# MariBax/self-supervised-depth-estimation

Measured on AMD Instinct MI355X. Metric: training images/sec at 192x640 bs12 (resnet18 depth+pose, 4-scale photometric+smoothness), higher is better.
Workload: dtype f32 (1x1 convolutions: bf16x3 split operands, fp32 accumulate); 1 GPU; BASELINE configs[1]: resnet18 depth+pose, 192x640, per-GPU batch 12, 4 scales, frames {0,-1,+1}, automasking, Adam lr 1e-4; random-init weights; global_batch=12, parallelism=dp1, tiebreak_noise=on-device counter RNG, setup_steps=0, step_launch=eager (one launch per kernel)

## Files before the change

### include/depthcore.h

```cpp
#ifndef DEPTHCORE_H
#define DEPTHCORE_H

#include <stddef.h>
#include <stdint.h>

#ifdef __cplusplus
extern "C" {
#endif

#define DC_OK 0
#define DC_EINVAL (-1)
#define DC_ELAUNCH (-2)
#define DC_EWORKSPACE (-3)
#define DC_EEMPTY (-4)

#define DC_MAX_SCALES 4

#define DC_OPT_NO_AUTOMASK 1u
#define DC_OPT_AVG_REPROJ 2u
#define DC_OPT_NO_SSIM 4u
#define DC_OPT_ALIGN_CORNERS 8u
#define DC_OPT_PRED_MASK 32u
#define DC_OPT_PHOTO_SPLIT 64u
#define DC_OPT_PHOTO_FULL 128u
// ... 312 lines not shown
} dc_attn_map;
typedef struct dc_attn_params {
    const float *wq, *bq, *wk, *bk, *wv, *bv, *rel_h, *rel_w;
} dc_attn_params;
int dc_attnconv_fwd(const dc_attn_map* x, const dc_attn_params* p, const dc_attn_map* res, float* y, int B, int C, int H, int W,
                    int relu_in, int relu_res, void* stream);
int dc_attnconv_param_count(int C);
size_t dc_attnconv_bwd_workspace(int B, int C, int H, int W);
int dc_attnconv_bwd(const dc_attn_map* x, const dc_attn_params* p, const dc_attn_map* res, const float* gy, const dc_attn_map* dx,
                    const float* dx_add, const dc_attn_map* dres, float* dparams, void* ws, int B, int C, int H, int W, int relu_in,
                    int relu_res, void* stream);

int dc_sasa_plan(int B, int C, int H, int W, int* plan);
int dc_sasa_fwd(const float* q, const float* k, const float* v, long long q_bstride, long long k_bstride, long long v_bstride,
                const float* rel_h, const float* rel_w, float* y, float* lse, int B, int C, int H, int W, void* stream);
size_t dc_sasa_bwd_workspace(int B, int C, int H, int W);
int dc_sasa_bwd(const float* q, const float* k, const float* v, long long q_bstride, long long k_bstride, long long v_bstride,
                const float* rel_h, const float* rel_w, const float* y, const float* lse, const float* gy, float* dq, float* dk,
                float* dv, float* drel_h, float* drel_w, void* ws, int B, int C, int H, int W, void* stream);

int dc_gru_rh_fwd(const float* gates, const float* h, float* rh, int B, int C, int P, void* stream);
int dc_gru_rh_bwd(const float* gates, const float* h, const float* g, float* d_gates, float* d_h, int B, int C, int P, void* stream);
int dc_gru_blend_fwd(const float* gates, const float* h, const float* cnm, float* h_next, int B, int C, int P, void* stream);
int dc_gru_blend_bwd(const float* gates, const float* h, const float* cnm, const float* g, float* d_gates, float* d_h, float* d_cnm,
                     int B, int C, int P, void* stream);
int dc_gru_rh_bwd_acc(const float* gates, const float* h, const float* g, float* d_gates, float* d_h, int B, int C, int P, void* stream);
int dc_gru_blend_bwd_acc(const float* gates, const float* h, const float* cnm, const float* g, float* d_gates, float* d_h, float* d_cnm,
                         int B, int C, int P, void* stream);
int dc_gather_copy(const float* const* src, float* const* dst, const size_t* n, int nseg, void* stream);
int dc_gru_residual_fwd(const float* f, const float* H, float* out, int n, size_t M, void* stream);
int dc_gru_residual_bwd(const float* g, float* d_H, int n, size_t M, void* stream);

typedef struct dc_gru_infer_level {
    const float* gates;
    const float* cnm;
    const float* f;
    float* h;
    float* rh;
    float* out;
    int32_t C, P;
} dc_gru_infer_level;
int dc_gru_infer_rh(const dc_gru_infer_level* lv, int nlev, int B, void* stream);
int dc_gru_infer_tail(const dc_gru_infer_level* lv, int nlev, int B, void* stream);
int dc_gru_infer_init(const float* const* h0, float* const* state, const size_t* M, int nlev, int B, void* stream);

enum { DC_PREC_F32 = 0, DC_PREC_BF16 = 1 };
int dc_set_matrix_precision(int precision);
int dc_get_matrix_precision(void);

int dc_set_wino_f4(int mode);
int dc_set_wino_persist(int mode);
#define DC_WINO_PHASE_DEFAULT (-3)
int dc_set_wino_phase(int mode);
int dc_set_dgrad_split(int mode);
int dc_wino_cache_new_owner(void);
int dc_wino_cache_register(int owner, const float* weight, int Ci, int Co);
int dc_wino_cache_release_owner(int owner);
int dc_wino_cache_refresh(int owner, void* stream);
int dc_wino_cache_invalidate(int owner);
int dc_wino_cache_clear(void);
int dc_wino_cache_variants(void);

#define DC_JITTER_NONE (-1)
#define DC_JITTER_BRIGHTNESS 0
#define DC_JITTER_CONTRAST 1
#define DC_JITTER_SATURATION 2
#define DC_JITTER_HUE 3
int dc_resample_ksize(int in_size, int out_size);
int dc_resample_table(int in_size, int out_size, int* bounds, int* kk);
int dc_data_resize_axis(const uint8_t* src, uint8_t* dst, int n_img, int Hi, int Wi, int out_size, int axis, const int* bounds,
                        const int* kk, int ksize, const uint8_t* flip, void* stream);
int dc_data_flip(const uint8_t* src, uint8_t* dst, int n_img, int H, int W, const uint8_t* flip, void* stream);
int dc_data_jitter(uint8_t* img, int n_img, int npix, const int* steps, const float* params, unsigned long long* sums, void* stream);
int dc_data_to_tensor(const uint8_t* img, float* out, int n_img, int npix, void* stream);
int dc_data_jitter_to_tensor(const uint8_t* img, float* color, float* color_aug, int n_img, int npix, const int* steps,
                             const float* params, unsigned long long* sums, void* stream);
int dc_data_to_rgbx(const uint8_t* img, float* out, int n_img, int npix, void* stream);
int dc_pack_rgbx(const float* x, float* out, int n_img, int npix, void* stream);
typedef struct dc_ragged_img {
    long long src_off, dst_off;
    int Hi, Wi, table, flip;
} dc_ragged_img;
typedef struct dc_ragged_table {
    int bounds_off, kk_off, ksize, in_size;
} dc_ragged_table;
int dc_data_ragged_resize_axis(const uint8_t* src, size_t src_bytes, uint8_t* dst, size_t dst_bytes, const dc_ragged_img* desc_host,
                               const dc_ragged_img* desc_dev, int n_img, int out_size, int axis, const dc_ragged_table* tab_host,
                               const dc_ragged_table* tab_dev, int n_tab, const int* bounds_host, const int* bounds_dev,
                               size_t bounds_len, const int* kk_dev, size_t kk_len, void* stream);
typedef struct dc_cached_img {
    long long slot_off;
    int flip, reserved;
} dc_cached_img;
int dc_data_cached_levels(const uint8_t* arena, size_t arena_bytes, const dc_cached_img* desc_host, const dc_cached_img* desc_dev,
                          int n_img, int height, int width, int num_scales, float* const* color, float* const* color_aug,
                          float* packed, const int* steps, const float* params, unsigned long long* sums, void* stream);
typedef struct dc_seq_plan {
    long long lds_bytes, table_len, scratch_bytes;
    int n_img, tail_start;
} dc_seq_plan;
int dc_data_seq_plan(int n, int H, int W, int S, int jitter, int lds_budget, dc_seq_plan* plan);
int dc_data_seq_levels(const uint8_t* frames, int n, int H, int W, int S, int flip, float* const* color, float* packed,
                       const int* steps, const float* params, const int* tab_host, const int* tab_dev, size_t tab_len,
                       void* scratch, size_t scratch_bytes, int lds_budget, void* stream);

#define DC_EVAL_TRAINER 0
// ... 53 lines not shown
```

### self-supervised-depth-estimation_amd/csrc/wino_wgrad.hip

```cpp
#include "dc_common.h"
#include "conv_bf16.h"
#include "conv_prof.h"
#include "wino.h"

#include <algorithm>

namespace dc {

using f4 = __attribute__((ext_vector_type(4))) float;
using f2w = __attribute__((ext_vector_type(2))) float;
using wrsrc_t = __amdgpu_buffer_rsrc_t;

constexpr int WG_MR = 4, WG_KR = 2;
constexpr int WG_KT = 16 * WG_KR;
constexpr int WG_GPS = 66;
constexpr int WG_XPS = 130;
constexpr int WINO_PHASES = 2;
constexpr int WG_SLAB = 4 * WG_MR * WG_KR * 4 * 3 * 64;

struct WinoWgArgs {
    const float* x; const float* gy; float* slab;
    int B, K, M, H, W;
    const float* x1;
    int C0, up0, pad;
    unsigned x1bytes;
    int RH, RW, GRS, XRS;
    int regs_x, regs_y, nsub;
    int splits, kblocks, mblocks;
    unsigned xbytes, gbytes;
    unsigned mg_nmk, mg_kblocks, mg_RW, mg_XPR, mg_per_img, mg_regs_x;
    unsigned long long* diag;
    const float* in_scale; const float* in_shift;
    int npg;
    int phase;
};
unsigned long long* wino_diag_ptr();

template <bool FUSED, int MR, int NG, int BNIN = 0>
__global__ __launch_bounds__(256 * NG, 2) void wino_wgrad_kernel(WinoWgArgs a) {
    static_assert(!(FUSED && BNIN), "the BatchNorm fold exists for the plain trunk launches");
    constexpr int KR = WG_KR, MT = 16 * MR, NGQ = MT / 8;
    constexpr int GL = MT * WG_GPS, XL = WG_KT * WG_XPS, GROUP_LDS = 2 * GL + 2 * XL;
    static_assert(NG == 1 || NG * GROUP_LDS >= 4 * MR * KR * 4 * 3 * 64, "the q exchange aliases the staging slabs");
    extern __shared__ float wg_smem[];
#ifdef WINO_DIAG
    const unsigned long long dg_start = __builtin_amdgcn_s_memtime(), dg_rstart = __builtin_amdgcn_s_memrealtime();
#endif
    const int lane = threadIdx.x & 63, wave_all = __builtin_amdgcn_readfirstlane(threadIdx.x >> 6);
    const int grp = NG == 1 ? 0 : wave_all >> 2, wave = wave_all & 3, tid = threadIdx.x & 255;
    int early = 0;
    if constexpr (NG == 2) {
        const int phase = a.phase < 0 ? (grp == 1 ? 0 : WINO_PHASES - 1) : a.phase;
        early = __builtin_amdgcn_readfirstlane(phase == 0 ? 1 : 0);
    }
    float* const gl0 = wg_smem + grp * GROUP_LDS;
    float* const xl0 = gl0 + 2 * GL;
    auto gl = [&](int buf) { return gl0 + buf * GL; };
    auto xl = [&](int buf) { return xl0 + buf * XL; };
    const int cl = lane & 15, tq = lane >> 4;
    const int H = a.H, W = a.W, RH = a.RH, RW = a.RW, GRS = a.GRS, XRS = a.XRS;
    const int nmk = a.mblocks * a.kblocks;
    const int lbid = xcd_logical_block(blockIdx.x, gridDim.x);
    const int split0 = fdiv(lbid, a.mg_nmk), mk = lbid - split0 * nmk;
    const int mb = fdiv(mk, a.mg_kblocks), kb = mk - mb * a.kblocks;
    const int per_img = a.regs_x * a.regs_y;
    const unsigned plane = (unsigned)(H * W) * 4u;
    const wrsrc_t gr = __builtin_amdgcn_make_buffer_rsrc(const_cast<float*>(a.gy), (short)0, (int)a.gbytes, 0x00020000);
    const wrsrc_t xr = __builtin_amdgcn_make_buffer_rsrc(const_cast<float*>(a.x), (short)0, (int)a.xbytes, 0x00020000);
    const wrsrc_t x1r = __builtin_amdgcn_make_buffer_rsrc(const_cast<float*>(FUSED ? a.x1 : a.x), (short)0,
                                                          (int)(FUSED ? a.x1bytes : a.xbytes), 0x00020000);
    const int C0 = FUSED ? a.C0 : a.K, up0 = FUSED ? a.up0 : 0;
    const unsigned plane0 = up0 ? (unsigned)((H >> 1) * (W >> 1)) * 4u : plane;

    const int gslot = tid & 31, gcg = tid >> 5;
    const int grow = fdiv(gslot, a.mg_RW), gcp = gslot - grow * RW;
    const bool g_in = gslot < 2 * RH * RW;
    const int glds = gcg * WG_GPS + grow * GRS + 2 * gcp;
    const int xslot = tid & 63, xcg = tid >> 6;
    const int XPR = RW + 2;
    const int xrow = fdiv(xslot, a.mg_XPR), xcp = xslot - xrow * XPR;
    const bool x_in = xslot < (2 * RH + 2) * XPR;
    const int xlds0 = xcg * WG_XPS + xrow * XRS + max(2 * xcp - 1, 0), xlds1 = xcg * WG_XPS + xrow * XRS + 2 * xcp;

    f2w pg[NGQ], px[8];
    bool px_ok = false;
    int px_grp = 0;
    float bsc[BNIN == 2 ? 2 : 1][BNIN ? 8 : 1], bsh[BNIN == 2 ? 2 : 1][BNIN ? 8 : 1];
    if constexpr (BNIN != 0) {
#pragma unroll
        for (int q = 0; q < 8; ++q) {
            const int chc = min(kb * WG_KT + wave + 4 * q, a.K - 1);
// ... 116 lines not shown
            for (int i = 0; i < MR; ++i) {
                if (i + 1 < MR) {
                    graw[(i + 1) & 1][0] = *reinterpret_cast<const f2w*>(gs_ + (i + 1) * 16 * WG_GPS + goffA[ks]);
                    graw[(i + 1) & 1][1] = *reinterpret_cast<const f2w*>(gs_ + (i + 1) * 16 * WG_GPS + goffB[ks]);
                }
                __builtin_amdgcn_sched_barrier(0);
                float r0 = fmaf(graw[i & 1][1].x, gs, graw[i & 1][0].x);
                float r1 = fmaf(graw[i & 1][1].y, gs, graw[i & 1][0].y);
                r0 = tv ? r0 : 0.f;
                r1 = tv ? r1 : 0.f;
                const float d1 = r0 + r1, d2 = r0 - r1;
#pragma unroll
                for (int j = 0; j < KR; ++j) {
                    acc[i][j][0] = __builtin_amdgcn_mfma_f32_16x16x4f32(r0, v[j][0], acc[i][j][0], 0, 0, 0);
                    acc[i][j][1] = __builtin_amdgcn_mfma_f32_16x16x4f32(d1, v[j][1], acc[i][j][1], 0, 0, 0);
                    acc[i][j][2] = __builtin_amdgcn_mfma_f32_16x16x4f32(d2, v[j][2], acc[i][j][2], 0, 0, 0);
                    acc[i][j][3] = __builtin_amdgcn_mfma_f32_16x16x4f32(r1, v[j][3], acc[i][j][3], 0, 0, 0);
                }
                __builtin_amdgcn_sched_barrier(0);
            }
        }
    };

    const int stride = NG * a.splits;
    int sub = split0 + grp * a.splits;
    if (sub < a.nsub) {
        prefetch(sub);
        commit(0);
        if (sub + stride < a.nsub) prefetch(sub + stride);
    }
    __syncthreads();
    if (early && sub + stride < a.nsub) {
        commit(1);
        if (sub + 2 * stride < a.nsub) prefetch(sub + 2 * stride);
    }
#ifdef WINO_DIAG
    const unsigned long long dg0 = __builtin_amdgcn_s_memtime();
#endif
    for (int it = 0, lead = split0; lead < a.nsub; lead += stride, sub += stride, ++it) {
        if (sub < a.nsub) compute(it & 1);
        if (early) __syncthreads();
        const int nxt = sub + (1 + early) * stride;
        if (nxt < a.nsub) {
            commit((it + 1 + early) & 1);
            if (nxt + stride < a.nsub) prefetch(nxt + stride);
        }
        if (!early) __syncthreads();
    }

#ifdef WINO_DIAG
    const unsigned long long dg1 = __builtin_amdgcn_s_memtime();
#endif
    const float sa = wave == 3 ? -1.f : 1.f;
    float* dst = a.slab + ((size_t)(split0 * nmk + mk) * 4 + wave) * (MR * KR * 4 * 3 * 64) + lane;
    float* ex = wg_smem + (size_t)wave * (MR * KR * 4 * 3 * 64) + lane;
    if (NG == 2 && grp == 1) {
#pragma unroll
        for (int i = 0; i < MR; ++i)
#pragma unroll
            for (int j = 0; j < KR; ++j)
#pragma unroll
                for (int r = 0; r < 4; ++r) {
                    const float u0 = sa * acc[i][j][0][r], u1 = sa * acc[i][j][1][r], u2 = sa * acc[i][j][2][r];
                    const float u3 = -sa * acc[i][j][3][r];
                    const float h = 0.5f * (u1 + u2);
                    float* d = ex + (((i * KR + j) * 4 + r) * 3) * 64;
                    d[0] = u0 + h;
                    d[64] = 0.5f * (u1 - u2);
                    d[128] = h + u3;
                }
    }
    if (NG == 2) __syncthreads();
    if (grp == 0) {
#pragma unroll
        for (int i = 0; i < MR; ++i)
#pragma unroll
            for (int j = 0; j < KR; ++j)
#pragma unroll
                for (int r = 0; r < 4; ++r) {
                    const float u0 = sa * acc[i][j][0][r], u1 = sa * acc[i][j][1][r], u2 = sa * acc[i][j][2][r];
                    const float u3 = -sa * acc[i][j][3][r];
                    const float h = 0.5f * (u1 + u2);
                    const int e = (((i * KR + j) * 4 + r) * 3) * 64;
                    float q0 = u0 + h, q1 = 0.5f * (u1 - u2), q2 = h + u3;
                    if (NG == 2) { q0 += ex[e]; q1 += ex[e + 64]; q2 += ex[e + 128]; }
                    dst[e] = q0;
                    dst[e + 64] = q1;
                    dst[e + 128] = q2;
                }
    }
#ifdef WINO_DIAG
    if (a.diag && lane == 0 && wave_all == 0) {
        __builtin_amdgcn_s_waitcnt(0x0f70);
        unsigned long long* o = a.diag + (size_t)blockIdx.x * 8;
        unsigned hwid, xcc;
        asm volatile("s_getreg_b32 %0, hwreg(HW_REG_HW_ID)" : "=s"(hwid));
        asm volatile("s_getreg_b32 %0, hwreg(HW_REG_XCC_ID)" : "=s"(xcc));
        o[1] = hwid; o[2] = xcc; o[3] = 0; o[4] = dg1 - dg0; o[5] = dg0 - dg_start;
        o[6] = __builtin_amdgcn_s_memtime() - dg1; o[7] = dg_rstart;
        o[0] = __builtin_amdgcn_s_memrealtime();
    }
#endif
}

constexpr int WR_GROUPS = 16;
__global__ __launch_bounds__(64 * WR_GROUPS) void wino_wreduce_kernel(const float* __restrict__ slab, float* __restrict__ dw,
                                                                      int splits, int nmk, int kblocks, int M, int K, int MR) {
    constexpr int KR = WG_KR;
    const size_t WAVE_SLAB = (size_t)MR * KR * 4 * 3 * 64;
    __shared__ float part[WR_GROUPS][12][64];
    const int lane = threadIdx.x & 63, grp = threadIdx.x >> 6;
    int e = blockIdx.x;
    const int r = e & 3; e >>= 2;
    const int j = e % KR; e /= KR;
    const int i = e % MR; e /= MR;
    const int mk = e;
    float q[4][3];
#pragma unroll
    for (int w = 0; w < 4; ++w)
#pragma unroll
        for (int c = 0; c < 3; ++c) q[w][c] = 0.f;
    const int groups = blockDim.x >> 6;
    const int per = (splits + groups - 1) / groups;
    const int s1 = min(splits, (grp + 1) * per);
    for (int s = grp * per; s < s1; ++s) {
        const float* src = slab + ((size_t)(s * nmk + mk) * 4) * WAVE_SLAB + (size_t)(((i * KR + j) * 4 + r) * 3) * 64 + lane;
#pragma unroll
        for (int w = 0; w < 4; ++w)
#pragma unroll
            for (int c = 0; c < 3; ++c) q[w][c] += src[(size_t)w * WAVE_SLAB + c * 64];
    }
#pragma unroll
    for (int w = 0; w < 4; ++w)
#pragma unroll
        for (int c = 0; c < 3; ++c) part[grp][w * 3 + c][lane] = q[w][c];
    __syncthreads();
    if (grp != 0) return;
#pragma unroll
    for (int w = 0; w < 4; ++w)
#pragma unroll
        for (int c = 0; c < 3; ++c) {
            float t = part[0][w * 3 + c][lane];
            for (int g = 1; g < groups; ++g) t += part[g][w * 3 + c][lane];
            q[w][c] = t;
        }
    const int mbk = mk / kblocks, kbk = mk - mbk * kblocks;
    const int m = mbk * (16 * MR) + i * 16 + (lane >> 4) * 4 + r, k = kbk * WG_KT + j * 16 + (lane & 15);
    if (m >= M || k >= K) return;
    float* out = dw + ((size_t)m * K + k) * 9;
#pragma unroll
    for (int c = 0; c < 3; ++c) {
        const float h = 0.5f * (q[1][c] + q[2][c]);
        out[0 + c] = q[0][c] + h;
        out[3 + c] = 0.5f * (q[1][c] - q[2][c]);
        out[6 + c] = h + q[3][c];
    }
}

__global__ __launch_bounds__(64 * WR_GROUPS) void wino_wreduce_col_kernel(const float* __restrict__ slab, float* __restrict__ dw,
                                                                      int splits, int nmk, int kblocks, int M, int K, int MR) {
    constexpr int KR = WG_KR;
    const size_t WAVE_SLAB = (size_t)MR * KR * 4 * 3 * 64;
    __shared__ float part[WR_GROUPS][4][64];
    const int lane = threadIdx.x & 63, grp = threadIdx.x >> 6;
    int e = blockIdx.x;
    const int c = e % 3; e /= 3;
    const int r = e & 3; e >>= 2;
    const int j = e % KR; e /= KR;
    const int i = e % MR; e /= MR;
    const int mk = e;
    float q[4] = {0.f, 0.f, 0.f, 0.f};
    const int groups = blockDim.x >> 6;
    const int per = (splits + groups - 1) / groups;
    const int s1 = min(splits, (grp + 1) * per);
    for (int s = grp * per; s < s1; ++s) {
        const float* src = slab + ((size_t)(s * nmk + mk) * 4) * WAVE_SLAB + (size_t)(((i * KR + j) * 4 + r) * 3 + c) * 64 + lane;
#pragma unroll
        for (int w = 0; w < 4; ++w) q[w] += src[(size_t)w * WAVE_SLAB];
    }
#pragma unroll
    for (int w = 0; w < 4; ++w) part[grp][w][lane] = q[w];
    __syncthreads();
    if (grp != 0) return;
#pragma unroll
    for (int w = 0; w < 4; ++w) {
        float t = part[0][w][lane];
        for (int g = 1; g < groups; ++g) t += part[g][w][lane];
        q[w] = t;
    }
    const int mbk = mk / kblocks, kbk = mk - mbk * kblocks;
    const int m = mbk * (16 * MR) + i * 16 + (lane >> 4) * 4 + r, k = kbk * WG_KT + j * 16 + (lane & 15);
    if (m >= M || k >= K) return;
    float* out = dw + ((size_t)m * K + k) * 9;
    const float h = 0.5f * (q[1] + q[2]);
    out[0 + c] = q[0] + h;
    out[3 + c] = 0.5f * (q[1] - q[2]);
    out[6 + c] = h + q[3];
}

static constexpr size_t wg_lds(int mr, int ng) { return (size_t)ng * (2 * 16 * mr * WG_GPS + 2 * WG_KT * WG_XPS) * sizeof(float); }

struct WgKernel { void (*fn)(WinoWgArgs); int threads; size_t lds; };
template <bool FUSED, int MR, int NG, int BNIN = 0>
static constexpr WgKernel wg_kernel() { return {wino_wgrad_kernel<FUSED, MR, NG, BNIN>, 256 * NG, wg_lds(MR, NG)}; }
enum { WG_ROW_FUSED = 3 };
static const WgKernel g_wg_kernels[4 * 3] = {
    wg_kernel<false, 4, 1>(), wg_kernel<false, 4, 2>(), wg_kernel<false, 2, 1>(),
    wg_kernel<false, 4, 1, 1>(), wg_kernel<false, 4, 2, 1>(), wg_kernel<false, 2, 1, 1>(),
    wg_kernel<false, 4, 1, 2>(), wg_kernel<false, 4, 2, 2>(), wg_kernel<false, 2, 1, 2>(),
    wg_kernel<true, 4, 1>(), wg_kernel<true, 4, 2>(), wg_kernel<true, 2, 1>(),
};

constexpr int WG_PHASE_SHIPPED = -1;
static bool wino_phase_valid(int m) { return m == DC_WINO_PHASE_DEFAULT || (m >= -1 && m < WINO_PHASES); }
static int g_wino_phase = [] {
    const char* f = getenv("DC_WINO_PHASE");
    const int v = f ? atoi(f) : DC_WINO_PHASE_DEFAULT;
    return wino_phase_valid(v) ? v : DC_WINO_PHASE_DEFAULT;
}();

struct WgPlan { int RH, RW, GRS, XRS, regs_x, regs_y, nsub, mblocks, kblocks, splits, mr, ng; };

static WgPlan wg_plan(int B, int Ci, int Co, int H, int W) {
    WgPlan p{};
    const int TH = ceil_div(H, 2), TW = W / 2;
    const int cand[3][4] = {{2, 8, 16, 20}, {4, 4, 8, 12}, {3, 5, 10, 14}};
    double best = -1.0;
    for (auto& c : cand) {
        const double util = (double)TH * TW / ((double)ceil_div(TH, c[0]) * ceil_div(TW, c[1]) * 16.0);
        if (util > best + 1e-9) { best = util; p.RH = c[0]; p.RW = c[1]; p.GRS = c[2]; p.XRS = c[3]; }
    }
    p.regs_x = ceil_div(TW, p.RW); p.regs_y = ceil_div(TH, p.RH); p.nsub = p.regs_x * p.regs_y * B;
    p.mr = (Co % 64 != 0 && Co % 64 <= 32) ? 2 : 4;
    if (const char* f = getenv("DC_WGRAD_MR")) { const int v = atoi(f); if (v == 2 || v == 4) p.mr = v; }
    p.mblocks = ceil_div(Co, 16 * p.mr); p.kblocks = ceil_div(Ci, WG_KT);
    const int nmk = p.mblocks * p.kblocks;
    p.ng = (p.mr == 4 && p.nsub >= 4 * ceil_div(256, nmk)) ? 2 : 1;
    if (const char* f = getenv("DC_WGRAD_NG")) { const int v = atoi(f); if (v == 1 || (v == 2 && p.mr == 4)) p.ng = v; }
    const int target = (p.mr == 2 && p.nsub >= 4096) ? 768 : 512 / p.ng;
    p.splits = std::max(1, std::min(std::max(1, p.nsub / (2 * p.ng)), ceil_div(target, nmk)));
    if (const char* f = getenv("DC_WGRAD_BLOCKS")) {
        const int tb = atoi(f);
        if (tb > 0) p.splits = std::max(1, std::min(std::max(1, p.nsub / (2 * p.ng)), ceil_div(tb, nmk)));
    }
    return p;
}

static int wg_launch(const float* x0, int C0, int up0, const float* x1, int C1, int pad, bool fused, const float* gy, float* dweight,
                     void* ws, int B, int Co, int H, int W, hipStream_t st, const dc_bn_fold* bn = nullptr) {
    const int Ci = C0 + C1;
    const size_t b0 = (size_t)B * C0 * (H >> up0) * (W >> up0) * 4, b1 = (size_t)B * C1 * H * W * 4, gb = (size_t)B * Co * H * W * 4;
    if (b0 >= 0x7fffffffull || b1 >= 0x7fffffffull || gb >= 0x7fffffffull) return DC_EINVAL;
    const WgPlan p = wg_plan(B, Ci, Co, H, W);
    WinoWgArgs a{};
    a.x = x0; a.x1 = x1; a.gy = gy; a.slab = (float*)ws; a.B = B; a.K = Ci; a.M = Co; a.H = H; a.W = W;
    a.C0 = C0; a.up0 = up0; a.pad = pad;
    a.RH = p.RH; a.RW = p.RW; a.GRS = p.GRS; a.XRS = p.XRS;
    a.regs_x = p.regs_x; a.regs_y = p.regs_y; a.nsub = p.nsub; a.splits = p.splits; a.kblocks = p.kblocks; a.mblocks = p.mblocks;
    a.xbytes = (unsigned)b0; a.x1bytes = (unsigned)b1; a.gbytes = (unsigned)gb;
    const int nmk = p.mblocks * p.kblocks, per_img = p.regs_x * p.regs_y;
    a.mg_nmk = fdiv_magic(nmk); a.mg_kblocks = fdiv_magic(p.kblocks); a.mg_RW = fdiv_magic(p.RW); a.mg_XPR = fdiv_magic(p.RW + 2);
    a.mg_per_img = fdiv_magic(per_img); a.mg_regs_x = fdiv_magic(p.regs_x);
    if ((unsigned long long)p.splits * nmk * (unsigned)nmk >= 0xffffffffull || (unsigned long long)p.nsub * (unsigned)per_img >= 0xffffffffull)
        return DC_EINVAL;
#ifdef WINO_DIAG
    a.diag = wino_diag_ptr();
#endif
    a.phase = g_wino_phase == DC_WINO_PHASE_DEFAULT ? WG_PHASE_SHIPPED : g_wino_phase;
    const bool bnin = bn && bn->in_scale;
    if (bnin) {
        if (fused || !bn->in_shift || bn->groups < 1 || bn->groups > 2 || B % bn->groups) return DC_EINVAL;
        a.in_scale = bn->in_scale; a.in_shift = bn->in_shift; a.npg = B / bn->groups;
    }
    static const bool attr = std::all_of(std::begin(g_wg_kernels), std::end(g_wg_kernels),
                                         [](const WgKernel& k) { return set_max_dynamic_lds(k.fn, k.lds); });
    if (!attr) return DC_ELAUNCH;
    const WgKernel& k = g_wg_kernels[3 * (fused ? WG_ROW_FUSED : (bnin ? bn->groups : 0)) + (p.mr == 4 ? p.ng - 1 : 2)];
    hipEvent_t pe = conv_prof_begin(PROF_WINO_WGRAD, 2.0 * B * (double)Co * Ci * 9.0 * H * W,
                                    2.0 * 16.0 * (double)p.nsub * 16.0 * (double)(p.mblocks * 16 * p.mr) * (p.kblocks * WG_KT),
                                    (double)b0 + (double)b1 + (double)gb + 36.0 * Co * Ci, st);
    hipLaunchKernelGGL(k.fn, dim3(p.splits * nmk), dim3(k.threads), k.lds, st, a);
    conv_prof_end(pe, st);
    DC_CHECK_LAUNCH();
    const int rblocks = nmk * p.mr * WG_KR * 4;
    const dim3 rthreads(64 * std::min(WR_GROUPS, std::max(1, p.splits / 2)));
    static const int colmode = [] { const char* f = getenv("DC_WREDUCE_COL"); return f ? atoi(f) : -1; }();
    if (colmode < 0 ? rblocks <= 1024 : colmode == 1)
        hipLaunchKernelGGL(wino_wreduce_col_kernel, dim3(rblocks * 3), rthreads, 0, st, (const float*)ws, dweight, p.splits, nmk, p.kblocks, Co, Ci, p.mr);
    else
        hipLaunchKernelGGL(wino_wreduce_kernel, dim3(rblocks), rthreads, 0, st, (const float*)ws, dweight, p.splits, nmk, p.kblocks, Co, Ci, p.mr);
    DC_CHECK_LAUNCH();
    return DC_OK;
}

size_t wino_wgrad_ws_bytes(int B, int Ci, int Co, int H, int W) {
    const WgPlan p = wg_plan(B, Ci, Co, H, W);
    return (size_t)p.splits * p.mblocks * p.kblocks * (WG_SLAB / WG_MR * p.mr) * sizeof(float);
}

int wino_wgrad_fused(const float* x0, int C0, int up0, const float* x1, int C1, int pad, const float* gp, float* dweight, void* ws,
                     int B, int Co, int H, int W, hipStream_t st) {
    return wg_launch(x0, C0, up0, x1, C1, pad, true, gp, dweight, ws, B, Co, H, W, st);
}

}

using namespace dc;

extern "C" int dc_set_wino_phase(int mode) {
    if (!wino_phase_valid(mode)) return DC_EINVAL;
    const int prev = g_wino_phase;
    g_wino_phase = mode;
    return prev;
}

extern "C" size_t dc_wino3x3_wgrad_workspace(int B, int Ci, int Co, int H, int W) {
    if (B <= 0 || Ci <= 0 || Co <= 0 || H <= 0 || W < 2 || (W & 1)) return 0;
    const size_t b16 = (size_t)c3b_wgrad_split(B, H, W, Co, Ci, 1) * Co * Ci * 9 * sizeof(float);
    return std::max(wino_wgrad_ws_bytes(B, Ci, Co, H, W), b16);
}

extern "C" int dc_wino3x3_wgrad(const float* x, const float* gy, float* dweight, void* ws, int B, int Ci, int Co, int H, int W,
                                void* stream) {
    if (!x || !gy || !dweight || !ws || B <= 0 || Ci <= 0 || Co <= 0 || H < 1 || W < 2 || (W & 1)) return DC_EINVAL;
    if (matrix_precision() == DC_PREC_BF16 && c3b_eligible(Ci, 0, 0, H, W, 1)) {
        const int sp = c3b_wgrad_split(B, H, W, Co, Ci, 1);
        const int rc = c3b_wgrad(x, Ci, 0, nullptr, 0, gy, (float*)ws, sp, B, Co, H, W, PAD_ZERO, 1, (hipStream_t)stream);
        return rc != DC_OK ? rc : conv_wreduce((const float*)ws, nullptr, dweight, nullptr, sp, Co * Ci * 9, 0, (hipStream_t)stream);
    }
    return wg_launch(x, Ci, 0, nullptr, 0, PAD_ZERO, false, gy, dweight, ws, B, Co, H, W, (hipStream_t)stream);
}

extern "C" int dc_wino3x3_wgrad_bn(const float* x, const float* gy, float* dweight, void* ws, int B, int Ci, int Co, int H, int W,
                                   const dc_bn_fold* bn, void* stream) {
    if (!bn || !bn->in_scale) return dc_wino3x3_wgrad(x, gy, dweight, ws, B, Ci, Co, H, W, stream);
    if (!x || !gy || !dweight || !ws || B <= 0 || Ci <= 0 || Co <= 0 || H < 1 || W < 2 || (W & 1)) return DC_EINVAL;
    if (matrix_precision() == DC_PREC_BF16 && c3b_eligible(Ci, 0, 0, H, W, 1)) return DC_EINVAL;
    return wg_launch(x, Ci, 0, nullptr, 0, PAD_ZERO, false, gy, dweight, ws, B, Co, H, W, (hipStream_t)stream, bn);
}
```

### self-supervised-depth-estimation_amd/depthcore/_lib.py

```python
import ctypes
import os
from ctypes import (POINTER, Structure, c_char_p, c_double, c_float, c_int, c_int32, c_size_t, c_uint8, c_uint32,
                    c_uint64, c_void_p)

import torch

_HERE = os.path.dirname(os.path.abspath(__file__))
PRODUCT_LIB = os.path.join(_HERE, "libdepthcore.so")
LIB_PATH = os.environ.get("DEPTHCORE_LIB") or PRODUCT_LIB
IS_VARIANT = os.path.realpath(LIB_PATH) != os.path.realpath(PRODUCT_LIB)
MAX_SCALES = 4

OPT_NO_AUTOMASK = 1
OPT_AVG_REPROJ = 2
OPT_NO_SSIM = 4
OPT_ALIGN_CORNERS = 8
OPT_NO_GRAD = 16
OPT_PRED_MASK = 32
OPT_PHOTO_SPLIT, OPT_PHOTO_FULL = 64, 128
PREC_F32, PREC_BF16 = 0, 1
PASS_FWD, PASS_DGRAD, PASS_WGRAD = 0, 1, 2

_ERR = {-1: "DC_EINVAL (bad shape / null pointer / unsupported option)",
        -2: "DC_ELAUNCH (hip launch failed)",
# ... 190 lines not shown
        "dc_stem_wgrad": (i, [p, i, f, f, p, p, p, i, i, i, i, p]),
        "dc_adam_chunk": (i, []),
        "dc_adam_step": (i, [p, p, p, p, i, f, c_double, c_double, f, p]),
        "dc_convs2_supported": (i, [i, i, i, i, i, i]),
        "dc_convs2_fwd_workspace": (z, [i, i, i, i, i, i]),
        "dc_convs2_fwd": (i, [p, p, p, p, i, i, i, i, i, i, p]),
        "dc_convs2_dgrad_workspace": (z, [i, i, i, i, i, i]),
        "dc_convs2_dgrad": (i, [p, p, p, p, i, i, i, i, i, i, p]),
        "dc_convs2_wgrad_workspace": (z, [i, i, i, i, i, i]),
        "dc_convs2_wgrad": (i, [p, p, p, p, i, i, i, i, i, i, p]),
        "dc_convs2_plan_query": (i, [i, i, i, i, i, i, i, POINTER(ConvS2Plan)]),
        "dc_conv2d_direct_fwd": (i, [p, p, p, p, i, i, i, i, i, i, i, i, p]),
        "dc_conv2d_direct_dgrad": (i, [p, p, p, i, i, i, i, i, i, i, i, p]),
        "dc_conv2d_direct_wgrad": (i, [p, p, p, p, i, i, i, i, i, i, i, i, p]),
        "dc_gru_rh_fwd": (i, [p, p, p, i, i, i, p]),
        "dc_gru_rh_bwd": (i, [p, p, p, p, p, i, i, i, p]),
        "dc_gru_blend_fwd": (i, [p, p, p, p, i, i, i, p]),
        "dc_gru_blend_bwd": (i, [p, p, p, p, p, p, p, i, i, i, p]),
        "dc_gru_rh_bwd_acc": (i, [p, p, p, p, p, i, i, i, p]),
        "dc_gru_blend_bwd_acc": (i, [p, p, p, p, p, p, p, i, i, i, p]),
        "dc_gather_copy": (i, [p, p, p, i, p]),
        "dc_gru_residual_fwd": (i, [p, p, p, i, z, p]),
        "dc_gru_residual_bwd": (i, [p, p, i, z, p]),
        "dc_gru_infer_rh": (i, [POINTER(GruInferLevel), i, i, p]),
        "dc_gru_infer_tail": (i, [POINTER(GruInferLevel), i, i, p]),
        "dc_gru_infer_init": (i, [p, p, p, i, i, p]),
        "dc_set_matrix_precision": (i, [i]),
        "dc_get_matrix_precision": (i, []),
        "dc_clear_error": (i, []),
        "dc_abort_capture": (i, [p]),
        "dc_set_gemm_split": (i, [i]),
        "dc_get_gemm_split": (i, []),
        "dc_gemm1x1x3_fwd_ok": (i, [i, i, i, i, i, i]),
        "dc_gemm1x1x3_dgrad_ok": (i, [i, i, i, i, i, i]),
        "dc_gemm1x1x3_workspace": (c_size_t, [i, i]),
        "dc_gemm1x1x3_fwd": (i, [p, p, p, p, p, i, i, i, i, i, i, i, p]),
        "dc_gemm1x1x3_dgrad": (i, [p, p, p, p, p, p, i, i, i, i, i, i, p]),
        "dc_gemm1x1x3_stat_parts": (i, [i, i, i, i, i, i, i, POINTER(c_int)]),
        "dc_gemm1x1x3_bwd_parts": (i, [i, i, i, i, i, i, POINTER(c_int)]),
        "dc_gemm1x1x3_wgrad_ok": (i, [i, i, i, i, i, i]),
        "dc_gemm1x1x3_wgrad_workspace": (c_size_t, [i, i, i, i, i, i]),
        "dc_gemm1x1x3_wgrad": (i, [p, p, p, p, i, i, i, i, i, i, p]),
        "dc_pointwise_workspace": (c_size_t, [i, POINTER(BnFold), i, i, i, i, i, i]),
        "dc_pointwise_stat_parts": (i, [i, i, i, i, i, i, i, POINTER(c_int)]),
        "dc_pointwise_bwd_parts": (i, [i, i, i, i, i, i, i, POINTER(c_int)]),
        "dc_pointwise_fwd": (i, [p, p, p, p, p, i, i, i, i, i, i, i, POINTER(BnFold), p]),
        "dc_pointwise_dgrad": (i, [p, p, p, p, p, p, i, i, i, i, i, i, POINTER(BnFold), p]),
        "dc_pointwise_wgrad": (i, [p, p, p, p, i, i, i, i, i, i, POINTER(BnFold), p]),
        "dc_set_photo_full": (i, [i]),
        "dc_get_photo_full": (i, []),
        "dc_set_wino_f4": (i, [i]),
        "dc_set_wino_persist": (i, [i]),
        "dc_set_wino_phase": (i, [i]),
        "dc_set_dgrad_split": (i, [i]),
        "dc_wino_cache_new_owner": (i, []),
        "dc_wino_cache_register": (i, [i, p, i, i]),
        "dc_wino_cache_release_owner": (i, [i]),
        "dc_wino_cache_refresh": (i, [i, p]),
        "dc_wino_cache_invalidate": (i, [i]),
        "dc_wino_cache_clear": (i, []),
        "dc_wino_cache_variants": (i, []),
        "dc_resample_ksize": (i, [i, i]),
        "dc_resample_table": (i, [i, i, p, p]),
        "dc_data_resize_axis": (i, [p, p, i, i, i, i, i, p, p, i, p, p]),
        "dc_data_flip": (i, [p, p, i, i, i, p, p]),
        "dc_data_jitter": (i, [p, i, i, p, p, p, p]),
        "dc_data_to_tensor": (i, [p, p, i, i, p]),
        "dc_data_to_rgbx": (i, [p, p, i, i, p]),
        "dc_pack_rgbx": (i, [p, p, i, i, p]),
        "dc_data_jitter_to_tensor": (i, [p, p, p, i, i, p, p, p, p]),
        "dc_data_ragged_resize_axis": (i, [p, z, p, z, p, p, i, i, i, p, p, i, p, p, z, p, z, p]),
        "dc_data_cached_levels": (i, [p, z, p, p, i, i, i, i, p, p, p, p, p, p, p]),
        "dc_data_seq_plan": (i, [i, i, i, i, i, i, POINTER(SeqPlan)]),
        "dc_data_seq_levels": (i, [p, i, i, i, i, i, p, p, p, p, p, p, z, p, z, i, p]),
        "dc_attnconv_fwd": (i, [POINTER(AttnMap), POINTER(AttnParams), POINTER(AttnMap), p, i, i, i, i, i, i, p]),
        "dc_attnconv_param_count": (i, [i]),
        "dc_attnconv_bwd_workspace": (z, [i, i, i, i]),
        "dc_attnconv_bwd": (i, [POINTER(AttnMap), POINTER(AttnParams), POINTER(AttnMap), p, POINTER(AttnMap), p, POINTER(AttnMap), p,
                                p, i, i, i, i, i, i, p]),
        "dc_sasa_plan": (i, [i, i, i, i, POINTER(c_int)]),
        "dc_sasa_fwd": (i, [p, p, p, ll, ll, ll, p, p, p, p, i, i, i, i, p]),
        "dc_sasa_bwd_workspace": (z, [i, i, i, i]),
        "dc_sasa_bwd": (i, [p, p, p, ll, ll, ll, p, p, p, p, p, p, p, p, p, p, p, i, i, i, i, p]),
        "dc_profile_enable": (i, [i]),
        "dc_profile_collect": (i, [POINTER(c_double), POINTER(c_int), POINTER(c_double), POINTER(c_int), POINTER(c_double),
                                   POINTER(c_double)]),
    }
    missing = []
    for name, (res, args) in S.items():
        try:
            fn = getattr(lib, name)
        except AttributeError:
            missing.append(name)
            continue
        fn.restype = res
        fn.argtypes = args
    return S, missing


EXPORTS = None
MISSING = None


def lib():
    global _lib, EXPORTS, MISSING
    if _lib is None:
# ... 40 lines not shown
```

Before: 1140 images/s.

## Apply Winograd wgrad output transform in-kernel, shrinking slab from 12 to 9 values

The Winograd weight-gradient kernel now applies the second (row) output transform inside the kernel. Each block's waves exchange their partial q values through LDS in pairs of M rows, so each block writes the final 9 3x3 taps per element instead of 12 per-wave partials. The split reduction kernels then simply sum 9 values and store them, which cuts slab traffic and workspace reads. The cost is extra LDS exchanges and barriers in the wgrad epilogue. The old layout stays available through an env var and a setter.

```diff
diff --git a/include/depthcore.h b/include/depthcore.h
--- a/include/depthcore.h
+++ b/include/depthcore.h
@@ -388,6 +388,7 @@
 int dc_set_wino_persist(int mode);
 #define DC_WINO_PHASE_DEFAULT (-3)
 int dc_set_wino_phase(int mode);
+int dc_set_wino_wgrad_gt(int mode);
 int dc_set_dgrad_split(int mode);
 int dc_wino_cache_new_owner(void);
 int dc_wino_cache_register(int owner, const float* weight, int Ci, int Co);
diff --git a/self-supervised-depth-estimation_amd/csrc/wino_wgrad.hip b/self-supervised-depth-estimation_amd/csrc/wino_wgrad.hip
--- a/self-supervised-depth-estimation_amd/csrc/wino_wgrad.hip
+++ b/self-supervised-depth-estimation_amd/csrc/wino_wgrad.hip
@@ -11,12 +11,15 @@
 using f2w = __attribute__((ext_vector_type(2))) float;
 using wrsrc_t = __amdgpu_buffer_rsrc_t;
 
-constexpr int WG_MR = 4, WG_KR = 2;
+constexpr int WG_KR = 2;
 constexpr int WG_KT = 16 * WG_KR;
 constexpr int WG_GPS = 66;
 constexpr int WG_XPS = 130;
 constexpr int WINO_PHASES = 2;
-constexpr int WG_SLAB = 4 * WG_MR * WG_KR * 4 * 3 * 64;
+__host__ __device__ constexpr int wg_block_slab(int mr, bool gt) { return mr * WG_KR * 4 * (gt ? 9 : 12) * 64; }
+__host__ __device__ constexpr int wg_slab_off(int mr, bool gt, int e4, int v) {
+    return gt ? (e4 * 9 + v) * 64 : (v / 3) * (wg_block_slab(mr, false) / 4) + (e4 * 3 + v % 3) * 64;
+}
 
 struct WinoWgArgs {
     const float* x; const float* gy; float* slab;
@@ -36,7 +39,7 @@
 };
 unsigned long long* wino_diag_ptr();
 
-template <bool FUSED, int MR, int NG, int BNIN = 0>
+template <bool FUSED, int MR, int NG, int BNIN = 0, bool GT = true>
 __global__ __launch_bounds__(256 * NG, 2) void wino_wgrad_kernel(WinoWgArgs a) {
     static_assert(!(FUSED && BNIN), "the BatchNorm fold exists for the plain trunk launches");
     constexpr int KR = WG_KR, MT = 16 * MR, NGQ = MT / 8;
@@ -259,42 +262,93 @@
     const unsigned long long dg1 = __builtin_amdgcn_s_memtime();
 #endif
     const float sa = wave == 3 ? -1.f : 1.f;
-    float* dst = a.slab + ((size_t)(split0 * nmk + mk) * 4 + wave) * (MR * KR * 4 * 3 * 64) + lane;
-    float* ex = wg_smem + (size_t)wave * (MR * KR * 4 * 3 * 64) + lane;
-    if (NG == 2 && grp == 1) {
-#pragma unroll
-        for (int i = 0; i < MR; ++i)
-#pragma unroll
-            for (int j = 0; j < KR; ++j)
-#pragma unroll
-                for (int r = 0; r < 4; ++r) {
-                    const float u0 = sa * acc[i][j][0][r], u1 = sa * acc[i][j][1][r], u2 = sa * acc[i][j][2][r];
-                    const float u3 = -sa * acc[i][j][3][r];
-                    const float h = 0.5f * (u1 + u2);
-                    float* d = ex + (((i * KR + j) * 4 + r) * 3) * 64;
-                    d[0] = u0 + h;
-                    d[64] = 0.5f * (u1 - u2);
-                    d[128] = h + u3;
+    if constexpr (GT) {
+        constexpr int IP = 2, EXW = IP * KR * 4 * 3 * 64;
+        static_assert(MR % IP == 0 && 4 * NG * EXW <= NG * GROUP_LDS, "the q exchange aliases the staging slabs");
+        float* const park = wg_smem + wave_all * EXW + lane;
+        float* const dst = a.slab + (size_t)(split0 * nmk + mk) * wg_block_slab(MR, true) + lane;
+#pragma unroll
+        for (int i0 = 0; i0 < MR; i0 += IP) {
+            if (i0) __syncthreads();
+#pragma unroll
+            for (int ii = 0; ii < IP; ++ii)
+#pragma unroll
+                for (int j = 0; j < KR; ++j)
+#pragma unroll
+                    for (int r = 0; r < 4; ++r) {
+                        const int i = i0 + ii;
+                        const float u0 = sa * acc[i][j][0][r], u1 = sa * acc[i][j][1][r], u2 = sa * acc[i][j][2][r];
+                        const float u3 = -sa * acc[i][j][3][r];
+                        const float h = 0.5f * (u1 + u2);
+                        float* d = park + (((ii * KR + j) * 4 + r) * 3) * 64;
+                        d[0] = u0 + h;
+                        d[64] = 0.5f * (u1 - u2);
+                        d[128] = h + u3;
+                    }
+            __syncthreads();
+#pragma unroll
+            for (int ii = 0; ii < IP; ++ii)
+#pragma unroll
+                for (int jj = 0; jj < (NG == 2 ? 1 : KR); ++jj) {
+                    const int j = NG == 2 ? grp : jj;
+                    const float* src = wg_smem + (((ii * KR + j) * 4 + wave) * 3) * 64 + lane;
+                    float o[9];
+#pragma unroll
+                    for (int c = 0; c < 3; ++c) {
+                        float sq[4];
+#pragma unroll
+                        for (int w = 0; w < 4; ++w) {
+                            sq[w] = src[w * EXW + c * 64];
+                            if (NG == 2) sq[w] += src[(4 + w) * EXW + c * 64];
+                        }
+                        const float h = 0.5f * (sq[1] + sq[2]);
+                        o[c] = sq[0] + h;
+                        o[3 + c] = 0.5f * (sq[1] - sq[2]);
+                        o[6 + c] = h + sq[3];
+                    }
+                    float* d = dst + wg_slab_off(MR, true, ((i0 + ii) * KR + j) * 4 + wave, 0);
+#pragma unroll
+                    for (int v = 0; v < 9; ++v) d[v * 64] = o[v];
                 }
-    }
-    if (NG == 2) __syncthreads();
-    if (grp == 0) {
-#pragma unroll
-        for (int i = 0; i < MR; ++i)
-#pragma unroll
-            for (int j = 0; j < KR; ++j)
-#pragma unroll
-                for (int r = 0; r < 4; ++r) {
-                    const float u0 = sa * acc[i][j][0][r], u1 = sa * acc[i][j][1][r], u2 = sa * acc[i][j][2][r];
-                    const float u3 = -sa * acc[i][j][3][r];
-                    const float h = 0.5f * (u1 + u2);
-                    const int e = (((i * KR + j) * 4 + r) * 3) * 64;
-                    float q0 = u0 + h, q1 = 0.5f * (u1 - u2), q2 = h + u3;
-                    if (NG == 2) { q0 += ex[e]; q1 += ex[e + 64]; q2 += ex[e + 128]; }
-                    dst[e] = q0;
-                    dst[e + 64] = q1;
-                    dst[e + 128] = q2;
-                }
+        }
+    } else {
+        float* dst = a.slab + ((size_t)(split0 * nmk + mk) * 4 + wave) * (wg_block_slab(MR, false) / 4) + lane;
+        float* ex = wg_smem + (size_t)wave * (wg_block_slab(MR, false) / 4) + lane;
+        if (NG == 2 && grp == 1) {
+#pragma unroll
+            for (int i = 0; i < MR; ++i)
+#pragma unroll
+                for (int j = 0; j < KR; ++j)
+#pragma unroll
+                    for (int r = 0; r < 4; ++r) {
+                        const float u0 = sa * acc[i][j][0][r], u1 = sa * acc[i][j][1][r], u2 = sa * acc[i][j][2][r];
+                        const float u3 = -sa * acc[i][j][3][r];
+                        const float h = 0.5f * (u1 + u2);
+                        float* d = ex + (((i * KR + j) * 4 + r) * 3) * 64;
+                        d[0] = u0 + h;
+                        d[64] = 0.5f * (u1 - u2);
+                        d[128] = h + u3;
+                    }
+        }
+        if (NG == 2) __syncthreads();
+        if (grp == 0) {
+#pragma unroll
+            for (int i = 0; i < MR; ++i)
+#pragma unroll
+                for (int j = 0; j < KR; ++j)
+#pragma unroll
+                    for (int r = 0; r < 4; ++r) {
+                        const float u0 = sa * acc[i][j][0][r], u1 = sa * acc[i][j][1][r], u2 = sa * acc[i][j][2][r];
+                        const float u3 = -sa * acc[i][j][3][r];
+                        const float h = 0.5f * (u1 + u2);
+                        const int e = (((i * KR + j) * 4 + r) * 3) * 64;
+                        float q0 = u0 + h, q1 = 0.5f * (u1 - u2), q2 = h + u3;
+                        if (NG == 2) { q0 += ex[e]; q1 += ex[e + 64]; q2 += ex[e + 128]; }
+                        dst[e] = q0;
+                        dst[e + 64] = q1;
+                        dst[e + 128] = q2;
+                    }
+        }
     }
 #ifdef WINO_DIAG
     if (a.diag && lane == 0 && wave_all == 0) {
@@ -311,86 +365,89 @@
 }
 
 constexpr int WR_GROUPS = 16;
+template <bool GT>
 __global__ __launch_bounds__(64 * WR_GROUPS) void wino_wreduce_kernel(const float* __restrict__ slab, float* __restrict__ dw,
                                                                       int splits, int nmk, int kblocks, int M, int K, int MR) {
-    constexpr int KR = WG_KR;
-    const size_t WAVE_SLAB = (size_t)MR * KR * 4 * 3 * 64;
-    __shared__ float part[WR_GROUPS][12][64];
+    constexpr int KR = WG_KR, NV = GT ? 9 : 12;
+    const size_t BLOCK_SLAB = wg_block_slab(MR, GT);
+    __shared__ float part[WR_GROUPS][NV][64];
     const int lane = threadIdx.x & 63, grp = threadIdx.x >> 6;
+    const int e4 = blockIdx.x % (MR * KR * 4);
     int e = blockIdx.x;
     const int r = e & 3; e >>= 2;
     const int j = e % KR; e /= KR;
     const int i = e % MR; e /= MR;
     const int mk = e;
-    float q[4][3];
-#pragma unroll
-    for (int w = 0; w < 4; ++w)
-#pragma unroll
-        for (int c = 0; c < 3; ++c) q[w][c] = 0.f;
+    float q[NV];
+#pragma unroll
+    for (int v = 0; v < NV; ++v) q[v] = 0.f;
     const int groups = blockDim.x >> 6;
     const int per = (splits + groups - 1) / groups;
     const int s1 = min(splits, (grp + 1) * per);
     for (int s = grp * per; s < s1; ++s) {
-        const float* src = slab + ((size_t)(s * nmk + mk) * 4) * WAVE_SLAB + (size_t)(((i * KR + j) * 4 + r) * 3) * 64 + lane;
-#pragma unroll
-        for (int w = 0; w < 4; ++w)
-#pragma unroll
-            for (int c = 0; c < 3; ++c) q[w][c] += src[(size_t)w * WAVE_SLAB + c * 64];
-    }
-#pragma unroll
-    for (int w = 0; w < 4; ++w)
-#pragma unroll
-        for (int c = 0; c < 3; ++c) part[grp][w * 3 + c][lane] = q[w][c];
+        const float* src = slab + (size_t)(s * nmk + mk) * BLOCK_SLAB + lane;
+#pragma unroll
+        for (int v = 0; v < NV; ++v) q[v] += src[wg_slab_off(MR, GT, e4, v)];
+    }
+#pragma unroll
+    for (int v = 0; v < NV; ++v) part[grp][v][lane] = q[v];
     __syncthreads();
     if (grp != 0) return;
 #pragma unroll
-    for (int w = 0; w < 4; ++w)
-#pragma unroll
-        for (int c = 0; c < 3; ++c) {
-            float t = part[0][w * 3 + c][lane];
-            for (int g = 1; g < groups; ++g) t += part[g][w * 3 + c][lane];
-            q[w][c] = t;
-        }
+    for (int v = 0; v < NV; ++v) {
+        float t = part[0][v][lane];
+        for (int g = 1; g < groups; ++g) t += part[g][v][lane];
+        q[v] = t;
+    }
     const int mbk = mk / kblocks, kbk = mk - mbk * kblocks;
     const int m = mbk * (16 * MR) + i * 16 + (lane >> 4) * 4 + r, k = kbk * WG_KT + j * 16 + (lane & 15);
     if (m >= M || k >= K) return;
     float* out = dw + ((size_t)m * K + k) * 9;
-#pragma unroll
-    for (int c = 0; c < 3; ++c) {
-        const float h = 0.5f * (q[1][c] + q[2][c]);
-        out[0 + c] = q[0][c] + h;
-        out[3 + c] = 0.5f * (q[1][c] - q[2][c]);
-        out[6 + c] = h + q[3][c];
-    }
-}
-
+    if constexpr (GT) {
+#pragma unroll
+        for (int v = 0; v < 9; ++v) out[v] = q[v];
+    } else {
+#pragma unroll
+        for (int c = 0; c < 3; ++c) {
+            const float h = 0.5f * (q[3 + c] + q[6 + c]);
+            out[0 + c] = q[c] + h;
+            out[3 + c] = 0.5f * (q[3 + c] - q[6 + c]);
+            out[6 + c] = h + q[9 + c];
+        }
+    }
+}
+
+template <bool GT>
 __global__ __launch_bounds__(64 * WR_GROUPS) void wino_wreduce_col_kernel(const float* __restrict__ slab, float* __restrict__ dw,
                                                                       int splits, int nmk, int kblocks, int M, int K, int MR) {
-    constexpr int KR = WG_KR;
-    const size_t WAVE_SLAB = (size_t)MR * KR * 4 * 3 * 64;
-    __shared__ float part[WR_GROUPS][4][64];
+    constexpr int KR = WG_KR, NV = GT ? 3 : 4;
+    const size_t BLOCK_SLAB = wg_block_slab(MR, GT);
+    __shared__ float part[WR_GROUPS][NV][64];
     const int lane = threadIdx.x & 63, grp = threadIdx.x >> 6;
     int e = blockIdx.x;
     const int c = e % 3; e /= 3;
+    const int e4 = e % (MR * KR * 4);
     const int r = e & 3; e >>= 2;
     const int j = e % KR; e /= KR;
     const int i = e % MR; e /= MR;
     const int mk = e;
-    float q[4] = {0.f, 0.f, 0.f, 0.f};
+    float q[NV];
+#pragma unroll
+    for (int w = 0; w < NV; ++w) q[w] = 0.f;
     const int groups = blockDim.x >> 6;
     const int per = (splits + groups - 1) / groups;
     const int s1 = min(splits, (grp + 1) * per);
     for (int s = grp * per; s < s1; ++s) {
-        const float* src = slab + ((size_t)(s * nmk + mk) * 4) * WAVE_SLAB + (size_t)(((i * KR + j) * 4 + r) * 3 + c) * 64 + lane;
-#pragma unroll
-        for (int w = 0; w < 4; ++w) q[w] += src[(size_t)w * WAVE_SLAB];
-    }
-#pragma unroll
-    for (int w = 0; w < 4; ++w) part[grp][w][lane] = q[w];
+        const float* src = slab + (size_t)(s * nmk + mk) * BLOCK_SLAB + wg_slab_off(MR, GT, e4, c) + lane;
+#pragma unroll
+        for (int w = 0; w < NV; ++w) q[w] += src[wg_slab_off(MR, GT, 0, 3 * w)];
+    }
+#pragma unroll
+    for (int w = 0; w < NV; ++w) part[grp][w][lane] = q[w];
     __syncthreads();
     if (grp != 0) return;
 #pragma unroll
-    for (int w = 0; w < 4; ++w) {
+    for (int w = 0; w < NV; ++w) {
         float t = part[0][w][lane];
         for (int g = 1; g < groups; ++g) t += part[g][w][lane];
         q[w] = t;
@@ -399,24 +456,40 @@
     const int m = mbk * (16 * MR) + i * 16 + (lane >> 4) * 4 + r, k = kbk * WG_KT + j * 16 + (lane & 15);
     if (m >= M || k >= K) return;
     float* out = dw + ((size_t)m * K + k) * 9;
-    const float h = 0.5f * (q[1] + q[2]);
-    out[0 + c] = q[0] + h;
-    out[3 + c] = 0.5f * (q[1] - q[2]);
-    out[6 + c] = h + q[3];
+    if constexpr (GT) {
+#pragma unroll
+        for (int b = 0; b < 3; ++b) out[3 * b + c] = q[b];
+    } else {
+        const float h = 0.5f * (q[1] + q[2]);
+        out[0 + c] = q[0] + h;
+        out[3 + c] = 0.5f * (q[1] - q[2]);
+        out[6 + c] = h + q[3];
+    }
 }
 
 static constexpr size_t wg_lds(int mr, int ng) { return (size_t)ng * (2 * 16 * mr * WG_GPS + 2 * WG_KT * WG_XPS) * sizeof(float); }
 
 struct WgKernel { void (*fn)(WinoWgArgs); int threads; size_t lds; };
-template <bool FUSED, int MR, int NG, int BNIN = 0>
-static constexpr WgKernel wg_kernel() { return {wino_wgrad_kernel<FUSED, MR, NG, BNIN>, 256 * NG, wg_lds(MR, NG)}; }
+template <bool GT, bool FUSED, int MR, int NG, int BNIN = 0>
+static constexpr WgKernel wg_kernel() { return {wino_wgrad_kernel<FUSED, MR, NG, BNIN, GT>, 256 * NG, wg_lds(MR, NG)}; }
 enum { WG_ROW_FUSED = 3 };
-static const WgKernel g_wg_kernels[4 * 3] = {
-    wg_kernel<false, 4, 1>(), wg_kernel<false, 4, 2>(), wg_kernel<false, 2, 1>(),
-    wg_kernel<false, 4, 1, 1>(), wg_kernel<false, 4, 2, 1>(), wg_kernel<false, 2, 1, 1>(),
-    wg_kernel<false, 4, 1, 2>(), wg_kernel<false, 4, 2, 2>(), wg_kernel<false, 2, 1, 2>(),
-    wg_kernel<true, 4, 1>(), wg_kernel<true, 4, 2>(), wg_kernel<true, 2, 1>(),
-};
+#define WG_KERNEL_TABLE(GT)                                                                                         \
+    {wg_kernel<GT, false, 4, 1>(),    wg_kernel<GT, false, 4, 2>(),    wg_kernel<GT, false, 2, 1>(),                \
+     wg_kernel<GT, false, 4, 1, 1>(), wg_kernel<GT, false, 4, 2, 1>(), wg_kernel<GT, false, 2, 1, 1>(),             \
+     wg_kernel<GT, false, 4, 1, 2>(), wg_kernel<GT, false, 4, 2, 2>(), wg_kernel<GT, false, 2, 1, 2>(),             \
+     wg_kernel<GT, true, 4, 1>(),     wg_kernel<GT, true, 4, 2>(),     wg_kernel<GT, true, 2, 1>()}
+static const WgKernel g_wg_kernels[2][4 * 3] = {WG_KERNEL_TABLE(false), WG_KERNEL_TABLE(true)};
+#undef WG_KERNEL_TABLE
+using WgReduce = void (*)(const float*, float*, int, int, int, int, int, int);
+static const WgReduce g_wg_reduce[2][2] = {{wino_wreduce_kernel<false>, wino_wreduce_col_kernel<false>},
+                                           {wino_wreduce_kernel<true>, wino_wreduce_col_kernel<true>}};
+
+constexpr int WG_GT_SHIPPED = 1;
+static int g_wino_wgrad_gt = [] {
+    const char* f = getenv("DC_WINO_WGRAD_GT");
+    const int v = f ? atoi(f) : WG_GT_SHIPPED;
+    return v == 0 || v == 1 ? v : WG_GT_SHIPPED;
+}();
 
 constexpr int WG_PHASE_SHIPPED = -1;
 static bool wino_phase_valid(int m) { return m == DC_WINO_PHASE_DEFAULT || (m >= -1 && m < WINO_PHASES); }
@@ -479,10 +552,11 @@
         if (fused || !bn->in_shift || bn->groups < 1 || bn->groups > 2 || B % bn->groups) return DC_EINVAL;
         a.in_scale = bn->in_scale; a.in_shift = bn->in_shift; a.npg = B / bn->groups;
     }
-    static const bool attr = std::all_of(std::begin(g_wg_kernels), std::end(g_wg_kernels),
+    static const bool attr = std::all_of(&g_wg_kernels[0][0], &g_wg_kernels[0][0] + 2 * 4 * 3,
                                          [](const WgKernel& k) { return set_max_dynamic_lds(k.fn, k.lds); });
     if (!attr) return DC_ELAUNCH;
-    const WgKernel& k = g_wg_kernels[3 * (fused ? WG_ROW_FUSED : (bnin ? bn->groups : 0)) + (p.mr == 4 ? p.ng - 1 : 2)];
+    const int gt = g_wino_wgrad_gt;
+    const WgKernel& k = g_wg_kernels[gt][3 * (fused ? WG_ROW_FUSED : (bnin ? bn->groups : 0)) + (p.mr == 4 ? p.ng - 1 : 2)];
     hipEvent_t pe = conv_prof_begin(PROF_WINO_WGRAD, 2.0 * B * (double)Co * Ci * 9.0 * H * W,
                                     2.0 * 16.0 * (double)p.nsub * 16.0 * (double)(p.mblocks * 16 * p.mr) * (p.kblocks * WG_KT),
                                     (double)b0 + (double)b1 + (double)gb + 36.0 * Co * Ci, st);
@@ -492,17 +566,16 @@
     const int rblocks = nmk * p.mr * WG_KR * 4;
     const dim3 rthreads(64 * std::min(WR_GROUPS, std::max(1, p.splits / 2)));
     static const int colmode = [] { const char* f = getenv("DC_WREDUCE_COL"); return f ? atoi(f) : -1; }();
-    if (colmode < 0 ? rblocks <= 1024 : colmode == 1)
-        hipLaunchKernelGGL(wino_wreduce_col_kernel, dim3(rblocks * 3), rthreads, 0, st, (const float*)ws, dweight, p.splits, nmk, p.kblocks, Co, Ci, p.mr);
-    else
-        hipLaunchKernelGGL(wino_wreduce_kernel, dim3(rblocks), rthreads, 0, st, (const float*)ws, dweight, p.splits, nmk, p.kblocks, Co, Ci, p.mr);
+    const bool col = colmode < 0 ? rblocks <= 1024 : colmode == 1;
+    hipLaunchKernelGGL(g_wg_reduce[gt][col], dim3(rblocks * (col ? 3 : 1)), rthreads, 0, st, (const float*)ws, dweight, p.splits, nmk, p.kblocks,
+                       Co, Ci, p.mr);
     DC_CHECK_LAUNCH();
     return DC_OK;
 }
 
 size_t wino_wgrad_ws_bytes(int B, int Ci, int Co, int H, int W) {
     const WgPlan p = wg_plan(B, Ci, Co, H, W);
-    return (size_t)p.splits * p.mblocks * p.kblocks * (WG_SLAB / WG_MR * p.mr) * sizeof(float);
+    return (size_t)p.splits * p.mblocks * p.kblocks * std::max(wg_block_slab(p.mr, false), wg_block_slab(p.mr, true)) * sizeof(float);
 }
 
 int wino_wgrad_fused(const float* x0, int C0, int up0, const float* x1, int C1, int pad, const float* gp, float* dweight, void* ws,
@@ -518,6 +591,13 @@
     if (!wino_phase_valid(mode)) return DC_EINVAL;
     const int prev = g_wino_phase;
     g_wino_phase = mode;
+    return prev;
+}
+
+extern "C" int dc_set_wino_wgrad_gt(int mode) {
+    if (mode != 0 && mode != 1) return DC_EINVAL;
+    const int prev = g_wino_wgrad_gt;
+    g_wino_wgrad_gt = mode;
     return prev;
 }
 
diff --git a/self-supervised-depth-estimation_amd/depthcore/_lib.py b/self-supervised-depth-estimation_amd/depthcore/_lib.py
--- a/self-supervised-depth-estimation_amd/depthcore/_lib.py
+++ b/self-supervised-depth-estimation_amd/depthcore/_lib.py
@@ -266,6 +266,7 @@
         "dc_set_wino_f4": (i, [i]),
         "dc_set_wino_persist": (i, [i]),
         "dc_set_wino_phase": (i, [i]),
+        "dc_set_wino_wgrad_gt": (i, [i]),
         "dc_set_dgrad_split": (i, [i]),
         "dc_wino_cache_new_owner": (i, []),
         "dc_wino_cache_register": (i, [i, p, i, i]),
```

Result: no change. 1136 images/s (-0.4%).
